# furcelay/gigalens

Hardware: AMD Instinct MI355X
Metric: forward+grad lens sims/sec, 128x128 px batch 1024; achieved HBM GB/s vs peak (higher is better)
Workload: dtype f32; 1 GPU; C2: EPL+shear lens, Sersic source, 128x128 px, batch 1024 per GPU, fp32 (BASELINE.json configs[1]); samples_per_gpu=1024, pixels=16384, z_dim=13, mode=fwdgrad, parallelism=single GPU

## Files before the change

gigalens_amd/csrc/gigalens_hip.hip:

```cpp
#include <algorithm>
#include <cmath>
#include <memory>
#include <cstdarg>
#include <cstdio>
#include <cstdlib>
#include <cstring>
#include <new>
#include <vector>

#include "gl_host_tables.h"
#include "gl_host.hip.h"
#include "gl_static.hip.h"
#include "gl_post.hip.h"
#include "gl_frontend.hip.h"
#include "gl_finalize.hip.h"

using namespace glk;

static thread_local char g_err[512] = "";

namespace glk {
int fail(int code, const char* fmt, ...) {
  va_list ap;
  va_start(ap, fmt);
  vsnprintf(g_err, sizeof(g_err), fmt, ap);
  va_end(ap);
  return code;
}
}

namespace {

int env_int(const char* name, int dflt) {
  const char* s = getenv(name);
  return (s && *s) ? atoi(s) : dflt;
}

void chunking(const gl_model* m, int B, int* chunk, int* n_chunks) {
  const long long tile_px = (long long)WG * 4;
  long long want = std::max<long long>((768 + B - 1) / B, ((long long)m->N + 8191) / 8192);
  if (m->target_wgs_set || !m->static_id) want = std::max<long long>(1, (m->target_wgs + B - 1) / B);
  long long per = ((long long)m->N + want - 1) / want;
  per = std::max(tile_px, (per + tile_px - 1) / tile_px * tile_px);
  if (m->chunk_px_override > 0) per = m->chunk_px_override;
  *chunk = (int)per;
  *n_chunks = (int)(((long long)m->N + per - 1) / per);
}

bool wave_front_end(const gl_model* m) { return m->has_epl && (int)m->comps.size() <= 64 && m->wave_prep; }
bool order_in_front_end(const gl_model* m, int B) {
  return wave_front_end(m) && m->use_order && m->order_fused && m->epl_comp >= 0 && B >= 2;
}

int tail_plan(const gl_model* m, int B, int n_chunks, int* tail_from, int* n_rows) {
  *tail_from = B;
  *n_rows = n_chunks;
  const bool pair_epl = m->pair && (m->static_id == ST_EPLSHEAR_SERSIC || m->static_id == ST_EPLSHEAR_SERSIC_SERSIC);
  if (m->tail_rows == 0 || !pair_epl || m->has_post || !order_in_front_end(m, B) || B > 1024) return 0;
  const int tiles = (m->N + 2 * WG - 1) / (2 * WG);
  const int slots = 256 * (m->static_id == ST_EPLSHEAR_SERSIC ? 3 : 2);
  int n_tail = m->tail_n, rows = m->tail_rows;
  if (n_tail < 0) {
    const long long wgs = (long long)B * n_chunks, rem = wgs % slots;
    if (wgs < slots || rem * 4 < slots) return 0;
    n_tail = (int)(rem / n_chunks);
  }
  if (rows < 0) rows = 2 * n_chunks;
  if (n_tail <= 0 || n_tail > B || rows > tiles || rows == n_chunks) return 0;
  *tail_from = B - n_tail;
  *n_rows = std::max(n_chunks, rows);
  return rows;
}

PostArgs post_args(const gl_model* m, float scale) {
  PostArgs p{};
  p.keff = m->d_psf;
  p.KH = m->KH; p.KW = m->KW; p.pt = m->pad_t; p.pl = m->pad_l;
  p.Hs = m->height; p.Ws = m->width; p.ss = m->supersample;
  p.H = m->height / m->supersample; p.W = m->width / m->supersample;
  p.scale = scale;
  return p;
}
constexpr bool corr_reachable(int kwp, int ncj, int ox) { return !(ox == 16 && kwp > 28) && !(ncj == 2 && kwp > 20); }
template <int KWP, int ST, int KS, int NCJ, int OX>
bool corr_launch(dim3 grid, size_t sh, hipStream_t stream, const float* in, float* out, const CorrArgs& a, std::atomic<const void*>* last) {
  if constexpr (corr_reachable(KWP, NCJ, OX)) {
    auto* fn = gl_corr_pair_kernel<KWP, ST, KS, NCJ, OX>;
    if (sh > 64 * 1024) {
      static const hipError_t big = hipFuncSetAttribute(reinterpret_cast<const void*>(fn), hipFuncAttributeMaxDynamicSharedMemorySize, 80 * 1024);
      if (big != hipSuccess) return false;
    }
    hipLaunchKernelGGL(fn, grid, dim3(CORR_GT * KS), sh, stream, in, out, a);
    if (last) last->store(reinterpret_cast<const void*>(fn), std::memory_order_relaxed);
    return true;
  } else {
    return false;
  }
}
bool launch_corr(const gl_model::CorrPlan& pl, int B, const float* in, float* out, float scale, hipStream_t stream, int dbg = 0,
                 int max_pairs_env = 0, int corr_wide = 1, std::atomic<const void*>* last = nullptr) {
  if (!pl.ok) return false;
  CorrArgs a = pl.args;
  a.B = B;
  a.scale = scale;
  a.dbg = dbg;
  a.vec = (a.Wi % 4 == 0 && a.Wout % 4 == 0 && ((reinterpret_cast<uintptr_t>(in) | reinterpret_cast<uintptr_t>(out)) & 15) == 0) ? 1 : 0;
  const bool wide = pl.ST == 2 && a.ncj == 1 && pl.KWP <= 28 && pl.max_KH <= 28 && corr_wide;
  const int ox = wide ? 16 : CORR_OX, ks = wide ? 8 : pl.ST == 2 ? 4 : 2;
  const int TR = (CORR_TR - 1) * pl.ST + pl.max_KH, TC = corr_tile_width((CORR_TCG * ox - 1) * pl.ST + pl.KWP) | 1;
  const size_t sh = std::max((size_t)TR * TC * sizeof(float2), (size_t)(ks - 1) * a.ncj * ox * CORR_GT * sizeof(float2) +
                                                                   (size_t)2 * CORR_TR * CORR_TCG * ox * a.ncj * sizeof(float));
  if (sh > (wide ? 80 : 64) * 1024) return false;
  const int max_pairs = max_pairs_env > 0 ? max_pairs_env : 65535 / a.n_class;
  if ((B + 1) / 2 > max_pairs) {
    for (int b_lo = 0; b_lo < B; b_lo += 2 * max_pairs) {
      const int nb = std::min(B - b_lo, 2 * max_pairs);
      if (!launch_corr(pl, nb, in + (size_t)b_lo * a.Hi * a.Wi, out + (size_t)b_lo * a.Hout * a.Wout, scale, stream, dbg, max_pairs_env, corr_wide, last)) return false;
    }
    return true;
  }
  const dim3 grid((pl.max_Wo + CORR_TCG * ox - 1) / (CORR_TCG * ox), (pl.max_Ho + CORR_TR - 1) / CORR_TR,
                  (unsigned)(a.n_class * ((B + 1) / 2)));
#define GL_CORR(KWP_, ST_, KS_, NCJ_, OX_) return corr_launch<KWP_, ST_, KS_, NCJ_, OX_>(grid, sh, stream, in, out, a, last);
#define GL_CORR_W(ST_, KS_, NCJ_, OX_)                                                                                          \
  switch (pl.KWP) {                                                                                                             \
    case 4: GL_CORR(4, ST_, KS_, NCJ_, OX_) case 8: GL_CORR(8, ST_, KS_, NCJ_, OX_) case 12: GL_CORR(12, ST_, KS_, NCJ_, OX_)     \
    case 16: GL_CORR(16, ST_, KS_, NCJ_, OX_) case 20: GL_CORR(20, ST_, KS_, NCJ_, OX_) case 24: GL_CORR(24, ST_, KS_, NCJ_, OX_) \
    case 28: GL_CORR(28, ST_, KS_, NCJ_, OX_) case 32: GL_CORR(32, ST_, KS_, NCJ_, OX_)                                          \
    default: return false;                                                                                                      \
  }
  if (wide) { GL_CORR_W(2, 8, 1, 16) }
  if (pl.ST == 2 && a.ncj == 1) { GL_CORR_W(2, 4, 1, CORR_OX) }
  if (pl.ST == 1 && a.ncj == 1) { GL_CORR_W(1, 2, 1, CORR_OX) }
  if (pl.ST == 1 && a.ncj == 2) { GL_CORR_W(1, 2, 2, CORR_OX) }
#undef GL_CORR_W
#undef GL_CORR
  return false;
}

}

namespace glk {

LaunchPlan launch_plan(const gl_model* m, int B) {
  LaunchPlan p{};
  chunking(m, B, &p.chunk, &p.n_chunks);
  p.tail_rows = tail_plan(m, B, p.n_chunks, &p.tail_from, &p.n_rows);
  return p;
}

Workspace carve(const gl_model* m, int B, void* base, const LaunchPlan& plan) {
  Workspace w{};
  size_t off = 0;
  char* p = (char*)base;
  w.derived = (float*)(p + off);
  off += align_up((size_t)B * m->D * sizeof(float), 256);
  w.partial = (float*)(p + off);
  off += align_up((size_t)B * plan.n_rows * m->A * sizeof(float), 256);
  w.params = (float*)(p + off);
  off += align_up((size_t)B * std::max(m->P, 1) * sizeof(float), 256);
  w.order = (int*)(p + off);
  off += align_up((size_t)B * sizeof(int), 256);
  w.cost = (int*)(p + off);
  off += align_up((size_t)B * sizeof(int), 256);
  if (m->G) {
    w.gal_dyn = (float*)(p + off);
    off += align_up((size_t)B * m->G * GM_ND * sizeof(float), 256);
  }
  if (m->pos_J) {
    auto take = [&](size_t n) { float* q = (float*)(p + off); off += align_up(n * sizeof(float), 256); return q; };
    w.pos_w = take((size_t)B * m->pos_J * 6);
    w.pos_adj = take((size_t)B * m->pos_J * 3);
    w.pos_g = take((size_t)B * m->pos_J * std::max(m->P, 1));
    w.pos_fam = take((size_t)B * m->pos_F * 2);
    w.pos_ll = take(B);
    w.pos_chi2 = take(B);
    w.pos_grad = take((size_t)B * std::max(m->P, 1));
  }
  if (m->has_post) {
    w.img_ss = (float*)(p + off);
    off += align_up((size_t)B * m->height * m->width * sizeof(float), 256);
    w.img_tmp = (float*)(p + off);
    off += align_up((size_t)B * (m->height / m->supersample) * (m->width / m->supersample) * sizeof(float), 256);
    w.stats = (float*)(p + off);
    off += align_up((size_t)B * 2 * sizeof(float), 256);
  } else if (m->mp_K >= 2) {
    w.img_tmp = (float*)(p + off);
    off += align_up((size_t)B * m->height * m->width * sizeof(float), 256);
    w.stats = (float*)(p + off);
    off += align_up((size_t)B * 2 * sizeof(float), 256);
  }
  w.bytes = off;
  return w;
}

MainArgs base_args(const gl_model* m, const Workspace& w, int chunk) {
  MainArgs a{};
  a.comps = m->d_comps;
  a.n_lens = m->n_lens;
  a.n_ll = m->n_ll;
  a.n_src = m->n_src;
// ... 415 lines not shown
    }
    cd.lin_off = (int)m->lin_cols.size();
    for (int k = 0; k < kind_num_linear(c.kind, iparam); ++k) m->lin_cols.push_back(p_off + kind_linear_col(c.kind, iparam) + k);
    if (c.kind == GL_USER_LIGHT && c.reserved == 1 && iparam >= 1) m->lin_cols.push_back(p_off + iparam - 1);
    p_off += cd.n_par;
    d_off += (kind_num_derived(c.kind, iparam) + 3) & ~3;
    a_off += cd.n_acc;
    m->comps.push_back(cd);
  }
  if (m->has_user && m->n_interp)
    return fail(GL_EUNSUPPORTED, "a model that mixes user-written profiles with GL_INTERPOL lights is not served: the run-time "
                                 "compiled kernels carry no image tables");
  m->P = p_off;
  for (int i = 0; i < n_lens; ++i) m->lens_params += m->comps[i].n_par;
  m->D = std::max(d_off, 4);
  m->A = a_off;
  m->Apad = a_off | 1;
  for (int i = 0; i < n_lens; ++i) m->has_nfw = m->has_nfw || m->comps[i].kind == K_NFW;
  m->nfw_lds = m->has_nfw ? sizeof(float) * 2 * glh::kNfwNodes : 0;
  m->ncols = ((size_t)(((m->D + 3) & ~3) + 64 * m->Apad) * sizeof(float) + m->nfw_lds <= 60 * 1024) ? 64 : 16;
  return GL_OK;
}

struct Knobs {
  int tile, tile_grad, use_static, pair, shp, cluster, corr_pair;
};
Knobs read_env_knobs(gl_model* m) {
  Knobs k{};
  k.tile = env_int("GIGALENS_HIP_TILE", 0);
  k.tile_grad = env_int("GIGALENS_HIP_TILE_GRAD", k.tile);
  k.use_static = env_int("GIGALENS_HIP_STATIC", 1);
  m->static_variant = env_int("GIGALENS_HIP_STATIC_VARIANT", 0);
  k.pair = env_int("GIGALENS_HIP_PAIR", 1);
  k.shp = env_int("GIGALENS_HIP_SHP", 1);
  k.cluster = env_int("GIGALENS_HIP_CLUSTER", -1);
  m->target_wgs = std::max(1, env_int("GIGALENS_HIP_TARGET_WGS", 2048));
  m->target_wgs_set = getenv("GIGALENS_HIP_TARGET_WGS") != nullptr;
  m->use_order = env_int("GIGALENS_HIP_ORDER", 1) != 0;
  m->order_fused = env_int("GIGALENS_HIP_ORDER_FUSED", 1) != 0;
  m->prep_lds = env_int("GIGALENS_HIP_PREP_LDS", 1) != 0;
  m->tail_rows = env_int("GIGALENS_HIP_TAIL_ROWS", -1);
  m->tail_n = env_int("GIGALENS_HIP_TAIL_N", -1);
#ifdef GL_EXPERIMENTS
  m->chunk_px_override = env_int("GIGALENS_HIP_CHUNK_PX", 0);
  m->dbg_flags = env_int("GIGALENS_HIP_DBGFLAGS", 0);
#endif
  m->shp_cull = env_int("GIGALENS_HIP_SHP_CULL", 1);
  m->shp_blocked = env_int("GIGALENS_HIP_SHP_BLOCKED", 1);
  m->corr_max_pairs = env_int("GIGALENS_HIP_CORR_MAXPAIRS", 0);
  m->corr_wide = env_int("GIGALENS_HIP_CORR_WIDE", 1);
  k.corr_pair = env_int("GIGALENS_HIP_CORR_PAIR", 1);
  m->wave_prep = env_int("GIGALENS_HIP_WAVE_PREP", 1) != 0;
  m->careful_tiles = env_int("GIGALENS_HIP_CAREFUL_TILES", 0) != 0;
  m->lstsq_wgs = std::max(1, env_int("GIGALENS_HIP_LSTSQ_WGS", 2048));
  m->lstsq_chol = env_int("GIGALENS_HIP_LSTSQ_CHOL", 1) != 0;
  m->lstsq_fused = env_int("GIGALENS_HIP_LSTSQ_FUSED", 1) != 0;
  return k;
}

int check_experiment_knobs(const gl_model* m) {
#ifdef GL_EXPERIMENTS
  if (m->chunk_px_override < 0 || m->chunk_px_override % (WG * 4) != 0)
    return fail(GL_EINVAL, "GIGALENS_HIP_CHUNK_PX=%d is not a positive multiple of the tile (%d pixels)", m->chunk_px_override, WG * 4);
  if (m->dbg_flags || m->chunk_px_override)
    fprintf(stderr, "libgigalens_hip: EXPERIMENT BUILD with GIGALENS_HIP_DBGFLAGS=%d GIGALENS_HIP_CHUNK_PX=%d -- results are not valid\n",
            m->dbg_flags, m->chunk_px_override);
#else
  (void)m;
  for (const char* name : {"GIGALENS_HIP_DBGFLAGS", "GIGALENS_HIP_CHUNK_PX"}) {
    const char* v = getenv(name);
    if (v && *v && atoi(v) != 0)
      return fail(GL_EINVAL, "%s is set but this library was built without -DGL_EXPERIMENTS (the dissection knobs do not exist in it)", name);
  }
#endif
  return GL_OK;
}

int select_kernels(gl_model* m, const Knobs& k) {
  const int n_comp = (int)m->comps.size(), n_lens = m->n_lens, n_lens_light = m->n_ll, n_src = m->n_src;
  m->tile = (k.tile == 4 || k.tile == 1) ? k.tile : 2;
  m->tile_grad = (k.tile_grad == 4 || k.tile_grad == 1 || k.tile_grad == 2) ? k.tile_grad : 0;
  m->static_id = k.use_static ? match_static(m) : 0;
  if (m->has_user) {
    m->static_id = 0;
    if (m->shp_big) return fail(GL_EUNSUPPORTED, "user-written profiles beside shapelets with n_max > %d", SH_CAP);
  }
  if (m->shp_big) {
    m->static_id = 0;
    if (m->fam)
      return fail(GL_EUNSUPPORTED, "shapelets with n_max > %d are served together with EPL / SIE / NFW / Shear / SIS lenses and Sersic "
                                   "lights only (this model also holds dPIE-family, catalogue, series or extended profiles)", SH_CAP);
  }
  m->pair = k.pair;
  int off = NSTAT;
  bool ok_row = true;
  for (int i = 0; i < n_comp; ++i) {
    ok_row = ok_row && m->comps[i].a_off == off;
    off += static_nacc(m->comps[i].kind);
  }
  if (m->pair && m->static_id && (!ok_row || off != m->A)) m->pair = 0;
  m->shp_kernel = k.shp && k.pair && m->static_id && ok_row && n_src == 1 && m->comps.back().kind == K_SHAPELETS;
  m->light_spherical = n_comp > n_lens;
  for (int i = n_lens; i < n_comp; ++i) m->light_spherical = m->light_spherical && m->comps[i].kind == K_SERSIC;
  m->static_matched = m->static_id;
  if (!m->tile_grad) m->tile_grad = m->static_id ? 1 : 2;
  if (!m->static_id) {
// ... 680 lines not shown
```

gigalens_amd/csrc/gl_launch.hip.h:

```cpp
#pragma once
#include <hip/hip_ext.h>

#include "gl_model.h"
#include "gl_static.hip.h"
#include "gl_pair.hip.h"
#include "gl_shp.hip.h"

namespace glk {

template <int MODE>
bool launch_static(const gl_model* m, const MainArgs& a, dim3 grid, dim3 block, size_t shmem, hipStream_t stream, hipEvent_t ev0, hipEvent_t ev1) {
  const int T = (MODE == IMG_BWD || MODE == LL_GRAD) ? m->tile_grad : m->tile;
#define GL_PAIR(WW, LK, CK, SK)                                                           \
  do {                                                                                    \
    m->last_main_fn = (const void*)&gl_pair_kernel<MODE, v2f, WW, LK, CK, SK>;            \
    hipExtLaunchKernelGGL((gl_pair_kernel<MODE, v2f, WW, LK, CK, SK>), grid, block, (std::uint32_t)(shmem), stream, ev0, ev1, 0, a); \
  } while (0)
  if (m->pair) {
    constexpr bool G = (MODE == IMG_BWD || MODE == LL_GRAD);
    constexpr int W1 = G ? 3 : 4, W2 = G ? 2 : 4;
    if (m->light_spherical) {
      switch (m->static_id) {
        case ST_EPLSHEAR_SERSIC: GL_PAIR(W1, L_EplShear, C_None, C_Sersic); return true;
        case ST_EPLSHEAR_SERSIC_SERSIC: GL_PAIR(W2, L_EplShear, C_Sersic, C_Sersic); return true;
        case ST_SIE_SERSIC: GL_PAIR(W1, L_Sie, C_None, C_Sersic); return true;
        case ST_SIESHEAR_SERSIC_SERSIC: GL_PAIR(W1, L_SieShear, C_Sersic, C_Sersic); return true;
        default: break;
      }
    } else {
      switch (m->static_id) {
        case ST_EPLSHEAR_SERSIC: GL_PAIR(W1, L_EplShear, C_None, C_SersicE); return true;
        case ST_EPLSHEAR_SERSIC_SERSIC: GL_PAIR(W2, L_EplShear, C_SersicE, C_SersicE); return true;
        case ST_SIE_SERSIC: GL_PAIR(W1, L_Sie, C_None, C_SersicE); return true;
        case ST_SIESHEAR_SERSIC_SERSIC: GL_PAIR(W2, L_SieShear, C_SersicE, C_SersicE); return true;
        default: break;
      }
    }
  }
#undef GL_PAIR
  if (m->shp_kernel && (m->static_id == ST_EPLSHEAR_SHAPELETS || m->static_id == ST_EPLSHEAR_SERSIC_SHAPELETS)) {
    constexpr int NPS = SH_SQ / 2;
    const size_t epi = (size_t)(16 * m->Apad + 4 * 16 * 17) * sizeof(float);
    const size_t sh = (size_t)((m->D + 3) & ~3) * sizeof(float) + std::max(shp_exchange_bytes(NPS), epi);
    const bool interp = (m->comps.back().flags & GL_FLAG_SHAPELETS_INTERPOLATE) != 0;
    const bool ragged = a.mask || a.pix || (a.N % (2 * WG)) != 0 || (a.chunk % (2 * WG)) != 0;
    MainArgs ab = a;
    ab.blk_w = (interp && !ragged && m->shp_blocked && m->width % 16 == 0 && m->height % 8 == 0 &&
                (long long)a.N == (long long)m->width * m->height) ? m->width : 0;
#define GL_SHP2(LLK_, I_, R_)                                                                                 \
  do {                                                                                                        \
    m->last_main_fn = (const void*)&gl_shp_kernel<MODE, 2, L_EplShear, LLK_, NPS, I_, R_>;                     \
    hipExtLaunchKernelGGL((gl_shp_kernel<MODE, 2, L_EplShear, LLK_, NPS, I_, R_>), grid, block, (std::uint32_t)(sh), stream, ev0, ev1, 0, ab);   \
  } while (0)
#define GL_SHP(LLK_, I_) do { if (ragged) GL_SHP2(LLK_, I_, true); else GL_SHP2(LLK_, I_, false); } while (0)
    if (m->static_id == ST_EPLSHEAR_SHAPELETS) { if (interp) GL_SHP(C_None, true); else GL_SHP(C_None, false); }
    else { if (interp) GL_SHP(C_SersicE, true); else GL_SHP(C_SersicE, false); }
#undef GL_SHP
#undef GL_SHP2
    return true;
  }
#define GL_LAUNCH(TT, WW, LK, CK, SK)                                                        \
  do {                                                                                       \
    m->last_main_fn = (const void*)&gl_static_kernel<MODE, TT, WW, LK, CK, SK>;              \
    hipExtLaunchKernelGGL((gl_static_kernel<MODE, TT, WW, LK, CK, SK>), grid, block, (std::uint32_t)(shmem), stream, ev0, ev1, 0, a); \
  } while (0)
  switch (m->static_id) {
    case ST_EPLSHEAR_SERSIC:
      if (T == 4) { if (m->static_variant == 2) GL_LAUNCH(4, 2, L_EplShear, C_None, C_Sersic); else GL_LAUNCH(4, 3, L_EplShear, C_None, C_Sersic); }
      else if (T == 1) GL_LAUNCH(1, 4, L_EplShear, C_None, C_Sersic);
      else { if (m->static_variant == 3) GL_LAUNCH(2, 3, L_EplShear, C_None, C_Sersic); else GL_LAUNCH(2, 4, L_EplShear, C_None, C_Sersic); }
      return true;
    case ST_EPLSHEAR_SERSIC_SERSIC:
      if (T == 4) GL_LAUNCH(4, 2, L_EplShear, C_Sersic, C_Sersic); else GL_LAUNCH(2, 4, L_EplShear, C_Sersic, C_Sersic);
// ... 52 lines not shown
```

gigalens_amd/csrc/gl_model.h:

```cpp
#pragma once
#include <hip/hip_runtime.h>

#include <atomic>
#include <string>
#include <utility>
#include <vector>

#include "../../include/gigalens_hip.h"
#include "gl_kernels.hip.h"

namespace glk {
__attribute__((visibility("hidden"))) int fail(int code, const char* fmt, ...);
}

#define GL_HIP(call)                                                                                   \
  do {                                                                                                 \
    hipError_t e_ = (call);                                                                            \
    if (e_ != hipSuccess) return glk::fail(GL_ELAUNCH, "%s failed: %s", #call, hipGetErrorString(e_)); \
  } while (0)

using glk::CompDesc;
using glk::CatDev;
using glk::SeriesDev;
using glk::InterpDev;
// ... 31 lines not shown
  operator T*() const { return p_; }

 private:
  T* p_ = nullptr;
};

struct CorrClass {
  int koff;
  int KH, pt, pl;
  int Ho, Wo[4];
  int oo_r, oo_c[4];
};
struct CorrArgs {
  const float* k;
  int n_class, ncj, B;
  int Hi, Wi;
  int Hout, Wout, os;
  float scale;
  int vec;
  int dbg;
  CorrClass cls[16];
};
}

struct gl_model {
  std::vector<CompDesc> comps;
  int n_lens = 0, n_ll = 0, n_src = 0;
  int P = 0, D = 0, A = 0, Apad = 0, ncols = 64;
  bool has_shapelets = false, has_table = false;
  bool shp_big = false;
  bool has_user = false;
  hipModule_t user_module = nullptr;
  hipFunction_t user_fn[5] = {nullptr, nullptr, nullptr, nullptr, nullptr};
  hipFunction_t user_pair_fn[4] = {nullptr, nullptr, nullptr, nullptr};
  std::string user_point_src;
  hipModule_t user_point_module = nullptr;
  hipFunction_t user_point_fn[7] = {nullptr, nullptr, nullptr, nullptr, nullptr, nullptr, nullptr};
  int height = 0, width = 0, supersample = 1, N = 0;
  float conversion_factor = 1.f;
  glk::DevBuf<CompDesc> d_comps;
  glk::DevBuf<float> d_gx;
  glk::DevBuf<float> d_gy;
  glk::DevBuf<int> d_pix;
  glk::DevBuf<float> d_shp_tab;
  glk::DevBuf<float> d_nfw_tab;
  int chunk_px_override = 0;
  int dbg_flags = 0;
  float grid_rmax = 0.f;
  int shp_blocked = 1;
  int shp_cull = 1;
  int corr_max_pairs = 0;
  int corr_wide = 1;
  int careful_tiles = 0;
  bool has_nfw = false;
  size_t nfw_lds = 0;
  int shp_stride = 0;
  glk::DevBuf<float> d_psf;
  struct CorrPlan { glk::CorrArgs args{}; int KWP = 0, ST = 0, max_Ho = 0, max_Wo = 0, max_KH = 0; bool ok = false; };
  CorrPlan corr_fwd, corr_bwd;
  glk::DevBuf<float> d_corr_k;
  int psf_h = 0, psf_w = 0;
  int KH = 1, KW = 1, pad_t = 0, pad_l = 0;
  bool has_post = false;
  int d_z = 0;
  glk::DevBuf<ZCol> d_zcols;
  glk::DevBuf<int> d_src;
  glk::DevBuf<float> d_const;
  int static_id = 0;
  int static_matched = 0;
  int static_variant = 0;
  int pair = 1;
  bool light_spherical = false;
  int cluster_w = 0;
  int cluster = 0;
  int pos_J = 0, pos_F = 0, lens_params = 0;
  glk::DevBuf<float> d_pos;
  glk::DevBuf<int> d_fam;
  std::vector<int> pos_fam_off;
  bool src_scaled = false;
  glk::DevBuf<float> d_src_scale;
  bool pos_scaled = false;
  glk::DevBuf<float> d_pos_scale;
  int mp_K = 0;
  glk::DevBuf<int> d_mp_lens;
  glk::DevBuf<float> d_mp_scale;
  bool pos_targets = false;
  glk::DevBuf<float> d_pos_target;
  int pos_n_flux = 0;
  glk::DevBuf<float> d_pos_flux;
  bool has_epl = false;
  int epl_comp = -1;
  int fam = 0;
  bool use_order = true;
  int tail_rows = -1, tail_n = -1;
  bool prep_lds = true;
  bool order_fused = true;
  bool wave_prep = true;
  int lstsq_wgs = 2048;
  bool lstsq_chol = true;
  bool lstsq_fused = true;
  int timing_slots = 0, timing_stride = 1;
  mutable std::atomic<long long> timing_count{0}, timing_calls{0};
  std::vector<hipEvent_t> evs;
  mutable std::atomic<const void*> last_main_fn{nullptr};
  mutable std::atomic<const void*> last_post_fn[2] = {{nullptr}, {nullptr}};
  mutable std::atomic<int> last_main_user{-1};
// ... 39 lines not shown
```

gigalens_amd/csrc/gl_pair.hip.h:

```cpp
#pragma once
#include "gl_static.hip.h"
#include "gl_vec.hip.h"

namespace glk {

#ifdef GL_HAVE_USER
template <class V, int CODE> __device__ __forceinline__ void user_mass_fwd_v(const float* d, V x, V y, V& bx, V& by) {
  constexpr unsigned body = (unsigned)user_code_body(CODE);
  if constexpr (sizeof(V) == sizeof(float)) {
    float ax, ay;
    glu::mass_fwd(body, d, x, y, ax, ay);
    bx -= ax; by -= ay;
  } else {
    float ax0, ay0, ax1, ay1;
    glu::mass_fwd(body, d, x.x, y.x, ax0, ay0);
    glu::mass_fwd(body, d, x.y, y.y, ax1, ay1);
    bx -= V{ax0, ax1};
    by -= V{ay0, ay1};
  }
}
template <class V, int CODE> __device__ __forceinline__ void user_mass_vjp_v(const float* d, V x, V y, V gx, V gy, V* acc) {
  constexpr unsigned body = (unsigned)user_code_body(CODE);
  constexpr int NPAR = user_code_npar(CODE);
  float t0[NPAR > 0 ? NPAR : 1], t1[NPAR > 0 ? NPAR : 1];
#pragma unroll
  for (int k = 0; k < NPAR; ++k) { t0[k] = 0.f; t1[k] = 0.f; }
  if constexpr (sizeof(V) == sizeof(float)) {
    glu::mass_vjp(body, d, x, y, gx, gy, t0);
#pragma unroll
    for (int k = 0; k < NPAR; ++k) acc[k] += t0[k];
  } else {
    glu::mass_vjp(body, d, x.x, y.x, gx.x, gy.x, t0);
    glu::mass_vjp(body, d, x.y, y.y, gx.y, gy.y, t1);
#pragma unroll
    for (int k = 0; k < NPAR; ++k) acc[k] += V{t0[k], t1[k]};
  }
}
template <class V, int CODE> __device__ __forceinline__ V user_light_fwd_v(const float* d, V x, V y) {
  constexpr unsigned body = (unsigned)user_code_body(CODE);
  if constexpr (sizeof(V) == sizeof(float)) return glu::light_fwd(body, d, x, y);
  else return V{glu::light_fwd(body, d, x.x, y.x), glu::light_fwd(body, d, x.y, y.y)};
}
template <class V, int CODE, bool SRC>
__device__ __forceinline__ void user_light_vjp_v(const float* d, V x, V y, V g, V* acc, V& gpx, V& gpy) {
  constexpr unsigned body = (unsigned)user_code_body(CODE);
  constexpr int NPAR = user_code_npar(CODE);
  float t0[NPAR > 0 ? NPAR : 1], t1[NPAR > 0 ? NPAR : 1];
#pragma unroll
  for (int k = 0; k < NPAR; ++k) { t0[k] = 0.f; t1[k] = 0.f; }
  if constexpr (sizeof(V) == sizeof(float)) {
    float dgx = 0.f, dgy = 0.f;
    glu::light_vjp(body, d, x, y, g, t0, dgx, dgy);
#pragma unroll
    for (int k = 0; k < NPAR; ++k) acc[k] += t0[k];
    if (SRC) { gpx += dgx; gpy += dgy; }
  } else {
    float dgx0 = 0.f, dgy0 = 0.f, dgx1 = 0.f, dgy1 = 0.f;
    glu::light_vjp(body, d, x.x, y.x, g.x, t0, dgx0, dgy0);
    glu::light_vjp(body, d, x.y, y.y, g.y, t1, dgx1, dgy1);
#pragma unroll
    for (int k = 0; k < NPAR; ++k) acc[k] += V{t0[k], t1[k]};
    if (SRC) { gpx += V{dgx0, dgx1}; gpy += V{dgy0, dgy1}; }
  }
}
#endif

template <int MODE, class V, int WAVES, class LK, class LLK, class SK>
__global__ void __launch_bounds__(WG, WAVES) gl_pair_kernel(MainArgs a) {
  constexpr int NL = LK::n, NLL = LLK::n, NS = SK::n, NLIGHT = NLL + NS;
  constexpr bool GRAD = (MODE == IMG_BWD || MODE == LL_GRAD);
  constexpr int W = sizeof(V) / sizeof(float);
  extern __shared__ float smem[];
  float* s_d = smem;
  float* s_acc = smem + ((a.D + 3) & ~3);
  const int tid = threadIdx.x;
  int rank = blockIdx.y, row = blockIdx.x, n_rows = gridDim.x, my_rows = gridDim.x;
  int p0 = row * a.chunk, p1 = min(p0 + a.chunk, a.N);
  if (a.tail_rows > 0) {
    n_rows = a.n_rows;
    if (rank >= a.tail_from) {
      const int j = (rank - a.tail_from) * (int)gridDim.x + row;
      rank = a.tail_from + j / a.tail_rows;
      if (rank >= a.n_samples) return;
      row = j % a.tail_rows;
      my_rows = a.tail_rows;
      const int tiles = (a.N + W * WG - 1) / (W * WG);
      p0 = (int)((long long)row * tiles / a.tail_rows) * (W * WG);
      p1 = min((int)((long long)(row + 1) * tiles / a.tail_rows) * (W * WG), a.N);
    }
  }
  const int b = a.order ? a.order[rank] : rank;
  const CompDesc* __restrict__ comps = a.comps;
  const float* __restrict__ gder = a.derived + (size_t)b * a.D;
  if (!GL_DBG(a.dbg, 4)) {
    if (a.D <= WG) {
      if (tid < a.D) s_d[tid] = gder[tid];
    } else {
      for (int i = tid; i < a.D; i += WG) s_d[i] = gder[i];
    }
  }
  __syncthreads();
  constexpr int NACC_L = [] { int n = 0; for (int i = 0; i < NL; ++i) n += static_nacc(LK::kinds[i]); return n; }();
  constexpr int NACC_C = [] {
    int n = 0;
    for (int i = 0; i < NLL; ++i) n += static_nacc(LLK::kinds[i]);
    for (int i = 0; i < NS; ++i) n += static_nacc(SK::kinds[i]);
    return n;
  }();
  V accL[NACC_L > 0 ? NACC_L : 1];
  V accC[NACC_C > 0 ? NACC_C : 1];
#pragma unroll
  for (int k = 0; k < NACC_L; ++k) accL[k] = V(0.f);
#pragma unroll
  for (int k = 0; k < NACC_C; ++k) accC[k] = V(0.f);
  V st0 = V(0.f), st1 = V(0.f);
  V wsum = V(0.f);
  int n_whole = 0;
  const float* dL[NL > 0 ? NL : 1];
  const float* dC[NLIGHT > 0 ? NLIGHT : 1];
#pragma unroll
  for (int i = 0; i < NL; ++i) dL[i] = s_d + comps[i].d_off;
#pragma unroll
  for (int i = 0; i < NLIGHT; ++i) dC[i] = s_d + comps[NL + i].d_off;
  const bool has_err = a.err != nullptr, has_mask = a.mask != nullptr, has_pix = a.pix != nullptr;
  auto plane = [](const float* p) { return __builtin_amdgcn_make_buffer_rsrc(const_cast<float*>(p), (short)0, -1, 0x00020000); };
  const auto r_obs = plane(a.obs), r_err = plane(a.err);

  auto tile = [&](int base, auto check_tag, auto err_tag) -> bool {
    constexpr bool CHECK = decltype(check_tag)::value;
    constexpr bool FAST = !CHECK;
    unsigned worst = 0;
    constexpr int ERR = decltype(err_tag)::value;
    const bool herr = ERR == 2 ? has_err : ERR == 1;
    unsigned jj[W], pidx[W];
    bool valid[W];
    V x, y, vmask = V(1.f);
#pragma unroll
    for (int w = 0; w < W; ++w) {
      int j = base + w * WG + tid;
      valid[w] = CHECK ? (j < p1) : true;
      jj[w] = (unsigned)(valid[w] ? j : p1 - 1);
      pidx[w] = (CHECK && has_pix) ? (unsigned)a.pix[jj[w]] : jj[w];
    }
    unsigned jo[W], po[W];
#pragma unroll
    for (int w = 0; w < W; ++w) { jo[w] = jj[w] << 2; po[w] = pidx[w] << 2; }
    auto ldf = [](const float* base, unsigned byte_off) { return *reinterpret_cast<const float*>(reinterpret_cast<const char*>(base) + byte_off); };
    auto ldb = [](auto rsrc, const float* base, unsigned byte_off) {
      if constexpr (CHECK) return *reinterpret_cast<const float*>(reinterpret_cast<const char*>(base) + byte_off);
      else return __uint_as_float(__builtin_amdgcn_raw_buffer_load_b32(rsrc, byte_off, 0, 0));
    };
    if constexpr (W == 2) {
      x = V{ldf(a.gx, jo[0]), ldf(a.gx, jo[1])};
      y = V{ldf(a.gy, jo[0]), ldf(a.gy, jo[1])};
      if (CHECK) vmask = V{valid[0] ? 1.f : 0.f, valid[1] ? 1.f : 0.f};
    } else {
      x = ldf(a.gx, jo[0]);
      y = ldf(a.gy, jo[0]);
      if (CHECK) vmask = valid[0] ? 1.f : 0.f;
    }
    V bx = x, by = y, m = V(0.f);
    EplStateV<V> est[NL > 0 ? NL : 1];
    SieStateV<V> sie_st[NL > 0 ? NL : 1];
    SerStateV<V> sst[NLIGHT > 0 ? NLIGHT : 1];
    static_for([&](auto I) {
      constexpr int i = decltype(I)::value;
      constexpr int kind = LK::kinds[i];
      if constexpr (kind == K_EPL) epl_fwd_v<V, GRAD, const float*, FAST>(dL[i], gder + comps[i].d_off, x, y, bx, by, est[i], &worst);
      else if constexpr (kind == K_SIE) sie_fwd_v<V>(dL[i], x, y, bx, by, (FAST && GRAD) ? &sie_st[i] : nullptr);
      else if constexpr (kind == K_SHEAR) shear_fwd_v<V>(dL[i], x, y, bx, by);
#ifdef GL_HAVE_USER
      else if constexpr (is_user_code(kind)) user_mass_fwd_v<V, kind>(dL[i], x, y, bx, by);
#endif
      else sis_fwd_v<V, FAST>(dL[i], x, y, bx, by, &worst);
    }, std::make_integer_sequence<int, NL>{});
    static_for([&](auto I) {
      constexpr int i = decltype(I)::value;
      constexpr bool src = i >= NLL;
      constexpr int lkind = src ? SK::kinds[src ? i - NLL : 0] : LLK::kinds[src ? 0 : i];
      constexpr bool ell = lkind != K_SERSIC;
#ifdef GL_HAVE_USER
      if constexpr (is_user_code(lkind)) m += user_light_fwd_v<V, lkind>(dC[i], src ? bx : x, src ? by : y);
      else
#endif
      m += sersic_fwd_v<V, ell, FAST>(dC[i], src ? bx : x, src ? by : y, sst[i], GRAD ? &worst : nullptr);
    }, std::make_integer_sequence<int, NLIGHT>{});
    auto nanp = m != m;
    if constexpr (FAST) {
      if ((__builtin_amdgcn_ballot_w64(worst > kGuardWidth) | __builtin_amdgcn_ballot_w64(any_nan(m))) != 0) return false;
      m = m * a.out_scale;
    } else {
      m = (nanp ? V(0.f) : m) * a.out_scale;
    }
    if (MODE == IMG_FWD) {
      float* row = a.img + (size_t)b * a.img_stride;
      if constexpr (W == 2) {
        if (valid[0]) row[pidx[0]] = m.x;
        if (valid[1]) row[pidx[1]] = m.y;
      } else {
        if (valid[0]) row[pidx[0]] = m;
      }
      return true;
    }
    V gm;
    if (MODE == IMG_BWD) {
      const float* row = a.gimg + (size_t)b * a.img_stride;
      V g;
      if constexpr (W == 2) g = V{row[pidx[0]], row[pidx[1]]}; else g = row[pidx[0]];
      gm = FAST ? g * a.out_scale : (nanp ? V(0.f) : (CHECK ? g * vmask : g) * a.out_scale);
    } else {
      V o, w = vmask, e = V(1.f);
      if constexpr (W == 2) {
        o = V{ldb(r_obs, a.obs, po[0]), ldb(r_obs, a.obs, po[1])};
        if (CHECK && has_mask) w = w * V{ldf(a.mask, po[0]), ldf(a.mask, po[1])};
        if (herr) e = V{ldb(r_err, a.err, po[0]), ldb(r_err, a.err, po[1])};
      } else {
        o = ldb(r_obs, a.obs, po[0]);
        if (CHECK && has_mask) w = w * ldf(a.mask, po[0]);
        if (herr) e = ldb(r_err, a.err, po[0]);
      }
      V dmo = m - o;
      V s2 = herr ? e * e : m * a.inv_t + a.bg2;
      V is2 = rcp(s2);
      V nm = log2_(s2);
      V c2 = __builtin_elementwise_fma(nm, V(0.f), dmo * dmo * is2);
      if (CHECK) {
        auto use = w != V(0.f);
        st0 += use ? c2 * w : V(0.f);
        st1 += use ? nm * w : V(0.f);
        wsum += w;
      } else {
        st0 += c2;
        st1 += nm;
      }
      if (MODE == LL_GRAD) {
        V g = herr ? -(dmo * is2) : (dmo * dmo * is2 - 1.f) * (is2 * (0.5f * a.inv_t)) - dmo * is2;
        gm = FAST ? g * a.out_scale : (nanp ? V(0.f) : (CHECK ? g * w : g) * a.out_scale);
      }
    }
    if constexpr (GRAD) {
      V gbx = V(0.f), gby = V(0.f);
      static_for([&](auto I) {
        constexpr int i = decltype(I)::value;
        constexpr bool src = i >= NLL;
        constexpr int off = [] {
          int n = 0;
          for (int j = 0; j < i; ++j) n += static_nacc(j < NLL ? LLK::kinds[j < NLL ? j : 0] : SK::kinds[j >= NLL ? j - NLL : 0]);
          return n;
        }();
        constexpr int lkind = src ? SK::kinds[src ? i - NLL : 0] : LLK::kinds[src ? 0 : i];
        constexpr bool ell = lkind != K_SERSIC;
#ifdef GL_HAVE_USER
        if constexpr (is_user_code(lkind)) user_light_vjp_v<V, lkind, src>(dC[i], src ? bx : x, src ? by : y, gm, accC + off, gbx, gby);
        else
#endif
        sersic_vjp_v<V, src, ell, FAST>(dC[i], sst[i], gm, accC + off, gbx, gby);
      }, std::make_integer_sequence<int, NLIGHT>{});
      gbx = -gbx;
      gby = -gby;
      static_for([&](auto I) {
        constexpr int i = decltype(I)::value;
        constexpr int kind = LK::kinds[i];
        constexpr int off = [] { int n = 0; for (int j = 0; j < i; ++j) n += static_nacc(LK::kinds[j]); return n; }();
        if constexpr (kind == K_EPL) epl_vjp_v<V>(dL[i], gbx, gby, est[i], accL + off);
        else if constexpr (kind == K_SIE) sie_vjp_v<V>(dL[i], x, y, gbx, gby, accL + off, FAST ? &sie_st[i] : nullptr);
        else if constexpr (kind == K_SHEAR) shear_vjp_v<V>(x, y, gbx, gby, accL + off);
#ifdef GL_HAVE_USER
        else if constexpr (is_user_code(kind)) user_mass_vjp_v<V, kind>(dL[i], x, y, gbx, gby, accL + off);
#endif
        else sis_vjp_v<V, FAST>(dL[i], x, y, gbx, gby, accL + off);
      }, std::make_integer_sequence<int, NL>{});
    }
    return true;
  };
  {
    bool sample_ok = !a.careful_tiles;
    static_for([&](auto I) {
      constexpr int i = decltype(I)::value;
      constexpr int lkind = i < NLL ? LLK::kinds[i < NLL ? i : 0] : SK::kinds[i >= NLL ? i - NLL : 0];
      if constexpr (!is_user_code(lkind)) sample_ok = sample_ok && sersic_fast_ok(gder + comps[NL + i].d_off);
    }, std::make_integer_sequence<int, NLIGHT>{});
    const bool plain = !has_mask && !has_pix && sample_ok;
    int base = p0;
    if (GL_DBG(a.dbg, 1)) base = p1;
    if (plain) {
      if (has_err) {
        for (; base + WG * W <= p1; base += WG * W, ++n_whole)
          if (!tile(base, std::false_type{}, std::integral_constant<int, 1>{})) break;
      } else {
        for (; base + WG * W <= p1; base += WG * W, ++n_whole)
          if (!tile(base, std::false_type{}, std::integral_constant<int, 0>{})) break;
      }
    }
    for (; base < p1; base += WG * W) tile(base, std::true_type{}, std::integral_constant<int, 2>{});
  }
  if (MODE == IMG_FWD) return;
  auto norm_term = [](float l2sum, float w) { return (l2sum + w * 2.6514961294723187f) * (float)kLn2; };
  float* out = a.partial + ((size_t)b * n_rows + row) * a.A;
  if (row == 0)
    for (int i = my_rows * a.A + tid; i < n_rows * a.A; i += WG) out[i] = 0.f;
  if (!GRAD) {
    for (int i = tid; i < 4 * a.Apad; i += WG) s_acc[i] = 0.f;
    __syncthreads();
  }
  if constexpr (GRAD) {
    constexpr int NV = NSTAT + NACC_L + NACC_C, NVP = (NV + 3) & ~3;
    float vals[NVP];
#pragma unroll
    for (int k = 0; k < NVP; ++k) vals[k] = 0.f;
    vals[0] = (MODE == LL_GRAD) ? hsum(st0) : 0.f;
    vals[1] = (MODE == LL_GRAD) ? norm_term(hsum(st1), hsum(wsum) + (float)(W * n_whole)) : 0.f;
    static_for([&](auto I) {
      constexpr int i = decltype(I)::value;
      constexpr int kind = LK::kinds[i];
      constexpr int off = [] { int n = 0; for (int j = 0; j < i; ++j) n += static_nacc(LK::kinds[j]); return n; }();
      constexpr int G = static_nacc(kind);
      float tmp[G];
#pragma unroll
      for (int k = 0; k < G; ++k) tmp[k] = hsum(accL[off + k]);
      if constexpr (kind == K_EPL) {
        tmp[EPLA_B] = tmp[EPLA_P0] * (dL[i][EPL_TM1] * dL[i][EPL_INVB]);
        tmp[EPLA_P0] *= rcp(dL[i][EPL_P0]);
        const float gxr = tmp[EPLA_CX], gyr = tmp[EPLA_CY], cc = dL[i][EPL_C], ss = dL[i][EPL_S];
        tmp[EPLA_CX] = -(gxr * cc - gyr * ss);
        tmp[EPLA_CY] = -(gxr * ss + gyr * cc);
      }
#pragma unroll
      for (int k = 0; k < G; ++k) vals[NSTAT + off + k] = tmp[k];
    }, std::make_integer_sequence<int, NL>{});
    static_for([&](auto I) {
      constexpr int i = decltype(I)::value;
      constexpr int off = [] {
        int n = 0;
        for (int j = 0; j < i; ++j) n += static_nacc(j < NLL ? LLK::kinds[j < NLL ? j : 0] : SK::kinds[j >= NLL ? j - NLL : 0]);
        return n;
      }();
      constexpr int lkind = i < NLL ? LLK::kinds[i < NLL ? i : 0] : SK::kinds[i >= NLL ? i - NLL : 0];
      if constexpr (is_user_code(lkind)) {
#pragma unroll
        for (int k = 0; k < static_nacc(lkind); ++k) vals[NSTAT + NACC_L + off + k] = hsum(accC[off + k]);
      } else {
#pragma unroll
        for (int k = 0; k < SER_NACC; ++k) vals[NSTAT + NACC_L + off + k] = hsum(accC[off + k]) * (k == SERA_INVN ? (float)kLn2 : 1.f);
      }
    }, std::make_integer_sequence<int, NLIGHT>{});
    const bool odd = tid & 1, hi = tid & 2;
    float* s_row16 = s_acc + (tid >> 4) * a.Apad;
#pragma unroll
    for (int g = 0; g < NVP / 4; ++g) {
      float r = quad_transpose_sum(vals[4 * g], vals[4 * g + 1], vals[4 * g + 2], vals[4 * g + 3], odd, hi);
      r = dpp_add(r, 0x114, 0xF);
      r = dpp_add(r, 0x118, 0xF);
      if ((tid & 15) >= 12 && 4 * g + (tid & 3) < NV) s_row16[4 * g + (tid & 3)] = r;
    }
    __syncthreads();
    for (int k = tid; k < NV; k += WG) {
      float v = 0.f;
#pragma unroll
      for (int j = 0; j < 16; ++j) v += s_acc[j * a.Apad + k];
      out[k] = v;
    }
    return;
  }
  float* s_row = s_acc + (tid >> 6) * a.Apad;
  const bool last_lane = (tid & 63) == 63;
  auto put = [&](float v, int idx) {
    if (!GL_DBG(a.dbg, 2)) v = wave_sum63(v);
    if (last_lane) s_row[idx] = v;
  };
  put((MODE == LL_FWD || MODE == LL_GRAD) ? hsum(st0) : 0.f, 0);
  put((MODE == LL_FWD || MODE == LL_GRAD) ? norm_term(hsum(st1), hsum(wsum) + (float)(W * n_whole)) : 0.f, 1);
  if (last_lane) { s_row[2] = 0.f; s_row[3] = 0.f; }
  __syncthreads();
  for (int k = tid; k < a.A; k += WG) {
    out[k] = (s_acc[k] + s_acc[a.Apad + k]) + (s_acc[2 * a.Apad + k] + s_acc[3 * a.Apad + k]);
  }
}

}
```

gigalens_amd/csrc/gl_static.hip.h:

```cpp
#pragma once
#if defined(__HIPCC_RTC__) && !__has_include(<utility>)
namespace std {
template <class T, T v> struct integral_constant {
  static constexpr T value = v;
  typedef T value_type;
  typedef integral_constant type;
  constexpr operator T() const { return v; }
};
typedef integral_constant<bool, true> true_type;
typedef integral_constant<bool, false> false_type;
template <class T, T... Is> struct integer_sequence {};
template <class T, T N> using make_integer_sequence = __make_integer_seq<integer_sequence, T, N>;
template <bool B, class T, class F> struct conditional { typedef T type; };
template <class T, class F> struct conditional<false, T, F> { typedef F type; };
template <bool B, class T, class F> using conditional_t = typename conditional<B, T, F>::type;
}
#else
#include <utility>
#endif

#include "gl_kernels.hip.h"
#include "gl_shapelets.hip.h"

namespace glk {
// ... 342 lines not shown
          }
        }
      }, std::make_integer_sequence<int, NL>{});
    }
  }
  if (MODE == IMG_FWD) return;
  const AccCol ac = acc_col(s_acc, a.Apad, a.ncols, tid);
  if (MODE == LL_FWD || MODE == LL_GRAD) wave_acc<2>(st, ac, 0);
  if constexpr (GRAD) {
    static_for([&](auto I) {
      constexpr int i = decltype(I)::value;
      constexpr int off = [] { int n = 0; for (int j = 0; j < i; ++j) n += static_nacc(LK::kinds[j]); return n; }();
      constexpr int G = static_nacc(LK::kinds[i]);
      float tmp[G];
#pragma unroll
      for (int k = 0; k < G; ++k) tmp[k] = accL[off + k];
      wave_acc<G>(tmp, ac, comps[i].a_off, comps[i].n_acc);
    }, std::make_integer_sequence<int, NL>{});
    static_for([&](auto I) {
      constexpr int i = decltype(I)::value;
      constexpr int kind = i < NLL ? LLK::kinds[i < NLL ? i : 0] : SK::kinds[i >= NLL ? i - NLL : 0];
      constexpr int off = [] {
        int n = 0;
        for (int j = 0; j < i; ++j) n += static_nacc(j < NLL ? LLK::kinds[j < NLL ? j : 0] : SK::kinds[j >= NLL ? j - NLL : 0]);
        return n;
      }();
      constexpr int G = static_nacc(kind);
      float tmp[G];
#pragma unroll
      for (int k = 0; k < G; ++k) tmp[k] = accC[off + k];
      wave_acc<G>(tmp, ac, comps[NL + i].a_off, comps[NL + i].n_acc);
    }, std::make_integer_sequence<int, NLIGHT>{});
  }
  __syncthreads();
  float* out = a.partial + ((size_t)b * gridDim.x + chunk) * a.A;
  for (int k = tid; k < a.A; k += WG) {
    float v = 0.f;
    for (int j = 0; j < a.ncols; ++j) v += s_acc[j * a.Apad + k];
    out[k] = v;
  }
}

using L_EplShear = KindList<K_EPL, K_SHEAR>;
using L_Sie = KindList<K_SIE>;
using L_SieShear = KindList<K_SIE, K_SHEAR>;
using C_None = KindList<>;
using C_Sersic = KindList<K_SERSIC>;
using C_SersicE = KindList<K_SERSIC_ELLIPSE>;
using C_Shapelets = KindList<K_SHAPELETS>;

enum StaticId { ST_NONE = 0, ST_EPLSHEAR_SERSIC, ST_EPLSHEAR_SERSIC_SERSIC, ST_SIE_SERSIC, ST_EPLSHEAR_SHAPELETS,
                ST_SIESHEAR_SERSIC_SERSIC, ST_EPLSHEAR_SERSIC_SHAPELETS  };


}
```

Baseline: 12.65 million sims/s.

## Add four-wave whole-tile pair kernel for EPL+shear Sersic gradient path

Adds a gradient-mode pair kernel variant (launch bounds 4 waves) for EPL+shear with a spherical Sersic source. It processes any leftover half tile with scalar float accumulators in two passes instead of the vector checked-tile loop. Launch planning now sizes chunks and the tail plan for 1024 resident slots when this variant applies. The aim is higher occupancy and better wave balance, at the cost of register pressure from the tighter launch bound and extra code paths.

```diff
diff --git a/gigalens_amd/csrc/gigalens_hip.hip b/gigalens_amd/csrc/gigalens_hip.hip
--- a/gigalens_amd/csrc/gigalens_hip.hip
+++ b/gigalens_amd/csrc/gigalens_hip.hip
@@ -36,9 +36,18 @@
   return (s && *s) ? atoi(s) : dflt;
 }
 
-void chunking(const gl_model* m, int B, int* chunk, int* n_chunks) {
+int resident_slots(const gl_model* m, bool whole4) {
+  if (whole4) return 256 * 4;
+  const bool two_waves = m->pair && m->static_id == ST_EPLSHEAR_SERSIC_SERSIC;
+  return 256 * (two_waves ? 2 : 3);
+}
+bool whole4_candidate(const gl_model* m) {
+  return m->pair && m->pair_whole4 && !m->has_post && !m->d_pix && pair_whole_serves(m->static_id, m->light_spherical);
+}
+
+void chunking(const gl_model* m, int B, int round_slots, int* chunk, int* n_chunks) {
   const long long tile_px = (long long)WG * 4;
-  long long want = std::max<long long>((768 + B - 1) / B, ((long long)m->N + 8191) / 8192);
+  long long want = std::max<long long>((round_slots + B - 1) / B, ((long long)m->N + 8191) / 8192);
   if (m->target_wgs_set || !m->static_id) want = std::max<long long>(1, (m->target_wgs + B - 1) / B);
   long long per = ((long long)m->N + want - 1) / want;
   per = std::max(tile_px, (per + tile_px - 1) / tile_px * tile_px);
@@ -52,13 +61,12 @@
   return wave_front_end(m) && m->use_order && m->order_fused && m->epl_comp >= 0 && B >= 2;
 }
 
-int tail_plan(const gl_model* m, int B, int n_chunks, int* tail_from, int* n_rows) {
+int tail_plan(const gl_model* m, int B, int n_chunks, int slots, int* tail_from, int* n_rows) {
   *tail_from = B;
   *n_rows = n_chunks;
   const bool pair_epl = m->pair && (m->static_id == ST_EPLSHEAR_SERSIC || m->static_id == ST_EPLSHEAR_SERSIC_SERSIC);
   if (m->tail_rows == 0 || !pair_epl || m->has_post || !order_in_front_end(m, B) || B > 1024) return 0;
   const int tiles = (m->N + 2 * WG - 1) / (2 * WG);
-  const int slots = 256 * (m->static_id == ST_EPLSHEAR_SERSIC ? 3 : 2);
   int n_tail = m->tail_n, rows = m->tail_rows;
   if (n_tail < 0) {
     const long long wgs = (long long)B * n_chunks, rem = wgs % slots;
@@ -143,10 +151,17 @@
 namespace glk {
 
 LaunchPlan launch_plan(const gl_model* m, int B) {
-  LaunchPlan p{};
-  chunking(m, B, &p.chunk, &p.n_chunks);
-  p.tail_rows = tail_plan(m, B, p.n_chunks, &p.tail_from, &p.n_rows);
-  return p;
+  auto plan_for = [&](bool whole4) {
+    LaunchPlan p{};
+    chunking(m, B, 256 * (whole4 ? 4 : 3), &p.chunk, &p.n_chunks);
+    p.tail_rows = tail_plan(m, B, p.n_chunks, resident_slots(m, whole4), &p.tail_from, &p.n_rows);
+    return p;
+  };
+  if (whole4_candidate(m)) {
+    const LaunchPlan p = plan_for(true);
+    if (pair_whole_shape(m->N, p.chunk)) return p;
+  }
+  return plan_for(false);
 }
 
 Workspace carve(const gl_model* m, int B, void* base, const LaunchPlan& plan) {
@@ -668,6 +683,7 @@
   k.corr_pair = env_int("GIGALENS_HIP_CORR_PAIR", 1);
   m->wave_prep = env_int("GIGALENS_HIP_WAVE_PREP", 1) != 0;
   m->careful_tiles = env_int("GIGALENS_HIP_CAREFUL_TILES", 0) != 0;
+  m->pair_whole4 = env_int("GIGALENS_HIP_PAIR_WHOLE4", 1) != 0;
   m->lstsq_wgs = std::max(1, env_int("GIGALENS_HIP_LSTSQ_WGS", 2048));
   m->lstsq_chol = env_int("GIGALENS_HIP_LSTSQ_CHOL", 1) != 0;
   m->lstsq_fused = env_int("GIGALENS_HIP_LSTSQ_FUSED", 1) != 0;
diff --git a/gigalens_amd/csrc/gl_launch.hip.h b/gigalens_amd/csrc/gl_launch.hip.h
--- a/gigalens_amd/csrc/gl_launch.hip.h
+++ b/gigalens_amd/csrc/gl_launch.hip.h
@@ -7,6 +7,9 @@
 #include "gl_shp.hip.h"
 
 namespace glk {
+
+template <int MODE>
+bool launch_pairw(const gl_model* m, const MainArgs& a, dim3 grid, dim3 block, size_t shmem, hipStream_t stream, hipEvent_t ev0, hipEvent_t ev1);
 
 template <int MODE>
 bool launch_static(const gl_model* m, const MainArgs& a, dim3 grid, dim3 block, size_t shmem, hipStream_t stream, hipEvent_t ev0, hipEvent_t ev1) {
@@ -19,6 +22,11 @@
   if (m->pair) {
     constexpr bool G = (MODE == IMG_BWD || MODE == LL_GRAD);
     constexpr int W1 = G ? 3 : 4, W2 = G ? 2 : 4;
+    if constexpr (G) {
+      if (m->pair_whole4 && !m->has_post && !a.mask && !a.pix && pair_whole_serves(m->static_id, m->light_spherical) &&
+          pair_whole_shape(a.N, a.chunk) && launch_pairw<MODE>(m, a, grid, block, shmem, stream, ev0, ev1))
+        return true;
+    }
     if (m->light_spherical) {
       switch (m->static_id) {
         case ST_EPLSHEAR_SERSIC: GL_PAIR(W1, L_EplShear, C_None, C_Sersic); return true;
diff --git a/gigalens_amd/csrc/gl_launch_pairw.hip.h b/gigalens_amd/csrc/gl_launch_pairw.hip.h
--- /dev/null
+++ b/gigalens_amd/csrc/gl_launch_pairw.hip.h
@@ -0,0 +1,23 @@
+#pragma once
+#include <hip/hip_ext.h>
+
+#include "gl_model.h"
+#include "gl_static.hip.h"
+#include "gl_pair.hip.h"
+
+namespace glk {
+
+template <int MODE>
+bool launch_pairw(const gl_model* m, const MainArgs& a, dim3 grid, dim3 block, size_t shmem, hipStream_t stream, hipEvent_t ev0, hipEvent_t ev1) {
+#define GL_PAIRW(LK, CK, SK)                                                              \
+  do {                                                                                    \
+    m->last_main_fn = (const void*)&gl_pairw_kernel<MODE, LK, CK, SK>;                    \
+    hipExtLaunchKernelGGL((gl_pairw_kernel<MODE, LK, CK, SK>), grid, block, (std::uint32_t)(shmem), stream, ev0, ev1, 0, a); \
+  } while (0)
+  if (m->static_id == ST_EPLSHEAR_SERSIC && m->light_spherical) GL_PAIRW(L_EplShear, C_None, C_Sersic);
+  else return false;
+#undef GL_PAIRW
+  return true;
+}
+
+}
diff --git a/gigalens_amd/csrc/gl_model.h b/gigalens_amd/csrc/gl_model.h
--- a/gigalens_amd/csrc/gl_model.h
+++ b/gigalens_amd/csrc/gl_model.h
@@ -107,6 +107,7 @@
   int corr_max_pairs = 0;
   int corr_wide = 1;
   int careful_tiles = 0;
+  int pair_whole4 = 1;
   bool has_nfw = false;
   size_t nfw_lds = 0;
   int shp_stride = 0;
diff --git a/gigalens_amd/csrc/gl_pair.hip.h b/gigalens_amd/csrc/gl_pair.hip.h
--- a/gigalens_amd/csrc/gl_pair.hip.h
+++ b/gigalens_amd/csrc/gl_pair.hip.h
@@ -65,11 +65,14 @@
 }
 #endif
 
-template <int MODE, class V, int WAVES, class LK, class LLK, class SK>
-__global__ void __launch_bounds__(WG, WAVES) gl_pair_kernel(MainArgs a) {
+template <class V> struct PairSums { V *L, *C, &st0, &st1, &wsum; };
+
+template <int MODE, class VK, bool WHOLE, class LK, class LLK, class SK>
+__device__ __forceinline__ void pair_body(const MainArgs& a) {
+  static_assert(!WHOLE || sizeof(VK) == 2 * sizeof(float), "the whole-tile form is a pair kernel");
   constexpr int NL = LK::n, NLL = LLK::n, NS = SK::n, NLIGHT = NLL + NS;
   constexpr bool GRAD = (MODE == IMG_BWD || MODE == LL_GRAD);
-  constexpr int W = sizeof(V) / sizeof(float);
+  constexpr int W = sizeof(VK) / sizeof(float);
   extern __shared__ float smem[];
   float* s_d = smem;
   float* s_acc = smem + ((a.D + 3) & ~3);
@@ -107,15 +110,16 @@
     for (int i = 0; i < NS; ++i) n += static_nacc(SK::kinds[i]);
     return n;
   }();
-  V accL[NACC_L > 0 ? NACC_L : 1];
-  V accC[NACC_C > 0 ? NACC_C : 1];
-#pragma unroll
-  for (int k = 0; k < NACC_L; ++k) accL[k] = V(0.f);
-#pragma unroll
-  for (int k = 0; k < NACC_C; ++k) accC[k] = V(0.f);
-  V st0 = V(0.f), st1 = V(0.f);
-  V wsum = V(0.f);
+  VK accL[NACC_L > 0 ? NACC_L : 1];
+  VK accC[NACC_C > 0 ? NACC_C : 1];
+#pragma unroll
+  for (int k = 0; k < NACC_L; ++k) accL[k] = VK(0.f);
+#pragma unroll
+  for (int k = 0; k < NACC_C; ++k) accC[k] = VK(0.f);
+  VK st0 = VK(0.f), st1 = VK(0.f);
+  VK wsum = VK(0.f);
   int n_whole = 0;
+  PairSums<VK> sums{accL, accC, st0, st1, wsum};
   const float* dL[NL > 0 ? NL : 1];
   const float* dC[NLIGHT > 0 ? NLIGHT : 1];
 #pragma unroll
@@ -126,7 +130,9 @@
   auto plane = [](const float* p) { return __builtin_amdgcn_make_buffer_rsrc(const_cast<float*>(p), (short)0, -1, 0x00020000); };
   const auto r_obs = plane(a.obs), r_err = plane(a.err);
 
-  auto tile = [&](int base, auto check_tag, auto err_tag) -> bool {
+  auto tile = [&](auto acc, int base, auto check_tag, auto err_tag) -> bool {
+    using V = std::remove_reference_t<decltype(acc.st0)>;
+    constexpr int W = sizeof(V) / sizeof(float);
     constexpr bool CHECK = decltype(check_tag)::value;
     constexpr bool FAST = !CHECK;
     unsigned worst = 0;
@@ -226,12 +232,12 @@
       V c2 = __builtin_elementwise_fma(nm, V(0.f), dmo * dmo * is2);
       if (CHECK) {
         auto use = w != V(0.f);
-        st0 += use ? c2 * w : V(0.f);
-        st1 += use ? nm * w : V(0.f);
-        wsum += w;
+        acc.st0 += use ? c2 * w : V(0.f);
+        acc.st1 += use ? nm * w : V(0.f);
+        acc.wsum += w;
       } else {
-        st0 += c2;
-        st1 += nm;
+        acc.st0 += c2;
+        acc.st1 += nm;
       }
       if (MODE == LL_GRAD) {
         V g = herr ? -(dmo * is2) : (dmo * dmo * is2 - 1.f) * (is2 * (0.5f * a.inv_t)) - dmo * is2;
@@ -251,10 +257,10 @@
         constexpr int lkind = src ? SK::kinds[src ? i - NLL : 0] : LLK::kinds[src ? 0 : i];
         constexpr bool ell = lkind != K_SERSIC;
 #ifdef GL_HAVE_USER
-        if constexpr (is_user_code(lkind)) user_light_vjp_v<V, lkind, src>(dC[i], src ? bx : x, src ? by : y, gm, accC + off, gbx, gby);
+        if constexpr (is_user_code(lkind)) user_light_vjp_v<V, lkind, src>(dC[i], src ? bx : x, src ? by : y, gm, acc.C + off, gbx, gby);
         else
 #endif
-        sersic_vjp_v<V, src, ell, FAST>(dC[i], sst[i], gm, accC + off, gbx, gby);
+        sersic_vjp_v<V, src, ell, FAST>(dC[i], sst[i], gm, acc.C + off, gbx, gby);
       }, std::make_integer_sequence<int, NLIGHT>{});
       gbx = -gbx;
       gby = -gby;
@@ -262,13 +268,13 @@
         constexpr int i = decltype(I)::value;
         constexpr int kind = LK::kinds[i];
         constexpr int off = [] { int n = 0; for (int j = 0; j < i; ++j) n += static_nacc(LK::kinds[j]); return n; }();
-        if constexpr (kind == K_EPL) epl_vjp_v<V>(dL[i], gbx, gby, est[i], accL + off);
-        else if constexpr (kind == K_SIE) sie_vjp_v<V>(dL[i], x, y, gbx, gby, accL + off, FAST ? &sie_st[i] : nullptr);
-        else if constexpr (kind == K_SHEAR) shear_vjp_v<V>(x, y, gbx, gby, accL + off);
+        if constexpr (kind == K_EPL) epl_vjp_v<V>(dL[i], gbx, gby, est[i], acc.L + off);
+        else if constexpr (kind == K_SIE) sie_vjp_v<V>(dL[i], x, y, gbx, gby, acc.L + off, FAST ? &sie_st[i] : nullptr);
+        else if constexpr (kind == K_SHEAR) shear_vjp_v<V>(x, y, gbx, gby, acc.L + off);
 #ifdef GL_HAVE_USER
-        else if constexpr (is_user_code(kind)) user_mass_vjp_v<V, kind>(dL[i], x, y, gbx, gby, accL + off);
+        else if constexpr (is_user_code(kind)) user_mass_vjp_v<V, kind>(dL[i], x, y, gbx, gby, acc.L + off);
 #endif
-        else sis_vjp_v<V, FAST>(dL[i], x, y, gbx, gby, accL + off);
+        else sis_vjp_v<V, FAST>(dL[i], x, y, gbx, gby, acc.L + off);
       }, std::make_integer_sequence<int, NL>{});
     }
     return true;
@@ -286,13 +292,33 @@
     if (plain) {
       if (has_err) {
         for (; base + WG * W <= p1; base += WG * W, ++n_whole)
-          if (!tile(base, std::false_type{}, std::integral_constant<int, 1>{})) break;
+          if (!tile(sums, base, std::false_type{}, std::integral_constant<int, 1>{})) break;
       } else {
         for (; base + WG * W <= p1; base += WG * W, ++n_whole)
-          if (!tile(base, std::false_type{}, std::integral_constant<int, 0>{})) break;
-      }
-    }
-    for (; base < p1; base += WG * W) tile(base, std::true_type{}, std::integral_constant<int, 2>{});
+          if (!tile(sums, base, std::false_type{}, std::integral_constant<int, 0>{})) break;
+      }
+    }
+    if constexpr (!WHOLE) {
+      for (; base < p1; base += WG * W) tile(sums, base, std::true_type{}, std::integral_constant<int, 2>{});
+    } else if (base < p1) {
+      float oneL[NACC_L > 0 ? NACC_L : 1], oneC[NACC_C > 0 ? NACC_C : 1], one0, one1, onew;
+      PairSums<float> one{oneL, oneC, one0, one1, onew};
+#pragma clang loop unroll(disable)
+      for (int half = 0; half < 2; ++half) {
+#pragma unroll
+        for (int k = 0; k < NACC_L; ++k) one.L[k] = sums.L[k].x;
+#pragma unroll
+        for (int k = 0; k < NACC_C; ++k) one.C[k] = sums.C[k].x;
+        one.st0 = sums.st0.x; one.st1 = sums.st1.x; one.wsum = sums.wsum.x;
+#pragma clang loop unroll(disable)
+        for (int t = base + half * WG; t < p1; t += WG * W) tile(one, t, std::true_type{}, std::integral_constant<int, 2>{});
+#pragma unroll
+        for (int k = 0; k < NACC_L; ++k) sums.L[k] = VK{sums.L[k].y, one.L[k]};
+#pragma unroll
+        for (int k = 0; k < NACC_C; ++k) sums.C[k] = VK{sums.C[k].y, one.C[k]};
+        sums.st0 = VK{sums.st0.y, one.st0}; sums.st1 = VK{sums.st1.y, one.st1}; sums.wsum = VK{sums.wsum.y, one.wsum};
+      }
+    }
   }
   if (MODE == IMG_FWD) return;
   auto norm_term = [](float l2sum, float w) { return (l2sum + w * 2.6514961294723187f) * (float)kLn2; };
@@ -377,4 +403,15 @@
   }
 }
 
-}
+template <int MODE, class V, int WAVES, class LK, class LLK, class SK>
+__global__ void __launch_bounds__(WG, WAVES) gl_pair_kernel(MainArgs a) {
+  pair_body<MODE, V, false, LK, LLK, SK>(a);
+}
+
+template <int MODE, class LK, class LLK, class SK>
+__global__ void __launch_bounds__(WG, 4) gl_pairw_kernel(MainArgs a) {
+  static_assert(MODE == IMG_BWD || MODE == LL_GRAD, "gl_pairw_kernel serves the gradient modes");
+  pair_body<MODE, v2f, true, LK, LLK, SK>(a);
+}
+
+}
diff --git a/gigalens_amd/csrc/gl_pairw_noslp_mode1.hip b/gigalens_amd/csrc/gl_pairw_noslp_mode1.hip
--- /dev/null
+++ b/gigalens_amd/csrc/gl_pairw_noslp_mode1.hip
@@ -0,0 +1,4 @@
+#include "gl_launch_pairw.hip.h"
+namespace glk {
+template bool launch_pairw<IMG_BWD>(const gl_model*, const MainArgs&, dim3, dim3, size_t, hipStream_t, hipEvent_t, hipEvent_t);
+}
diff --git a/gigalens_amd/csrc/gl_pairw_noslp_mode3.hip b/gigalens_amd/csrc/gl_pairw_noslp_mode3.hip
--- /dev/null
+++ b/gigalens_amd/csrc/gl_pairw_noslp_mode3.hip
@@ -0,0 +1,4 @@
+#include "gl_launch_pairw.hip.h"
+namespace glk {
+template bool launch_pairw<LL_GRAD>(const gl_model*, const MainArgs&, dim3, dim3, size_t, hipStream_t, hipEvent_t, hipEvent_t);
+}
diff --git a/gigalens_amd/csrc/gl_static.hip.h b/gigalens_amd/csrc/gl_static.hip.h
--- a/gigalens_amd/csrc/gl_static.hip.h
+++ b/gigalens_amd/csrc/gl_static.hip.h
@@ -418,5 +418,12 @@
 enum StaticId { ST_NONE = 0, ST_EPLSHEAR_SERSIC, ST_EPLSHEAR_SERSIC_SERSIC, ST_SIE_SERSIC, ST_EPLSHEAR_SHAPELETS,
                 ST_SIESHEAR_SERSIC_SERSIC, ST_EPLSHEAR_SERSIC_SHAPELETS  };
 
-
-}
+inline bool pair_whole_serves(int static_id, bool light_spherical) {
+  return static_id == ST_EPLSHEAR_SERSIC && light_spherical;
+}
+constexpr int kPairWholeMinTiles = 8;
+inline bool pair_whole_shape(int N, int chunk) {
+  return N % (2 * WG) == 0 && chunk % (2 * WG) == 0 && N / (2 * WG) >= kPairWholeMinTiles;
+}
+
+}
```

New measurement: 12.52 million sims/s. 1.0% lower.
